# aperezhortal/pySPEEDY

Hardware: AMD Instinct MI355X
Metric: simulated-years/day (whole node), T30L8 (higher is better)
Workload: dtype f64

## Files before the change

### pyspeedy_amd/csrc/coupler_point.hpp

```cpp
#pragma once
#include <hip/hip_runtime.h>

#include "stream_store.hpp"
#include "surface.hpp"

namespace spd {

struct CouplerArgs {
    SurfacePtrs S;
    TimeInterp w;
    int first, count, day, land_coupling, sst_anomaly, anom_planes, fresh;
};

namespace cpl {
constexpr int NGc = IX * IL;
__device__ constexpr double SBCd = 5.67e-8f, ALHCd = 2501.0f, EMISFCd = 0.98f, ALBSEAd = 0.07f, ALBICEd = 0.60f;

__device__ inline double forin5(const double *f12, size_t p, const TimeInterp &w) {
    return w.w5[0] * f12[p + static_cast<size_t>(NGc) * w.m5[0]] + w.w5[1] * f12[p + static_cast<size_t>(NGc) * w.m5[1]] +
           w.w5[2] * f12[p + static_cast<size_t>(NGc) * w.m5[2]] + w.w5[3] * f12[p + static_cast<size_t>(NGc) * w.m5[3]] +
           w.w5[4] * f12[p + static_cast<size_t>(NGc) * w.m5[4]];
}
__device__ inline double forint(const double *f12, size_t p, const TimeInterp &w) {
    const double a = f12[p + static_cast<size_t>(NGc) * w.l0];
    const double d = w.wlin * (f12[p + static_cast<size_t>(NGc) * w.l1] - a);
    return a + d;
}
}


__device__ __forceinline__ void coupler_point(const SurfacePtrs &S, int mem, int p, const TimeInterp &w, int day, int land_coupling,
                                              int sst_anomaly, int anom_planes, int fresh) {
    using namespace cpl;
    constexpr int NG = NGc;
    const size_t o = static_cast<size_t>(mem) * NG + p, o12 = static_cast<size_t>(mem) * 12 * NG + p;
    double stlcl;
    if (fresh) {
        stlcl = forin5(S.stl12, o12, w);
        const double snowdcl = forint(S.snowd12, o12, w);
        const double soilwcl = forint(S.soilw12, o12, w);
        stream_store(&S.stlcl_obs[o], stlcl);
        stream_store(&S.snowdcl_obs[o], snowdcl);
        stream_store(&S.soilwcl_obs[o], soilwcl);
        stream_store(&S.snow_depth[o], snowdcl);
        stream_store(&S.soil_avail_water[o], soilwcl);
    } else {
        stlcl = S.stlcl_obs[o];
    }
    if (day == 0) {
        stream_store(&S.stl_lm[o], stlcl);
        stream_store(&S.land_temp[o], stlcl);
    } else if (land_coupling) {
        double tanom = S.stl_lm[o] - stlcl;
        tanom = S.cdland[o] * (tanom + S.rhcapl[o] * S.hfluxn[static_cast<size_t>(mem) * 3 * NG + p]);
        const double stl = tanom + stlcl;
        stream_store(&S.stl_lm[o], stl);
        stream_store(&S.land_temp[o], stl);
    } else if (fresh) {
        stream_store(&S.land_temp[o], stlcl);
    }

    const double sstfr = 273.2f - 1.8f;
    double sstcl, sicecl, ticecl, sstan_ob = S.sstan_ob[o];
    if (fresh) {
        sstcl = forin5(S.sst12, o12, w);
        sicecl = forint(S.sea_ice_frac12, o12, w);
        if (sst_anomaly) {
            const size_t oa = static_cast<size_t>(mem) * anom_planes * NG + p;
            const double a = S.sst_anom[oa + static_cast<size_t>(NG) * w.a0];
            const double da = w.wan * (S.sst_anom[oa + static_cast<size_t>(NG) * w.a1] - a);
            sstan_ob = a + da;
            stream_store(&S.sstan_ob[o], sstan_ob);
        }
        if (sstcl > sstfr) {
            sicecl = fmin(0.5, sicecl);
            ticecl = sstfr;
            if (sicecl > 0.0) sstcl = sstfr + (sstcl - sstfr) / (1.0f - sicecl);
        } else {
            sicecl = fmax(0.5, sicecl);
            ticecl = sstfr + (sstcl - sstfr) / sicecl;
            sstcl = sstfr;
        }
        stream_store(&S.sstcl_ob[o], sstcl);
        stream_store(&S.sicecl_ob[o], sicecl);
        stream_store(&S.ticecl_ob[o], ticecl);
    } else {
        sstcl = S.sstcl_ob[o];
        sicecl = S.sicecl_ob[o];
        ticecl = S.ticecl_ob[o];
    }
    double sst_om, tice_om, sice_om;
    if (day == 0) {
        sst_om = 0.0;
        tice_om = ticecl;
        sice_om = sicecl;
    } else {
        const double tice_am = S.tice_am[o], sice_am = S.sice_am[o];
        const double hfl2 = S.hfluxn[static_cast<size_t>(mem) * 3 * NG + NG + p];
        tice_om = S.tice_om[o];
        sst_om = S.sst_om[o];
        const double s4 = (sstfr * sstfr) * (sstfr * sstfr), t4 = (tice_am * tice_am) * (tice_am * tice_am);
        const double difice = (ALBSEAd - ALBICEd) * S.ssrd[o] + EMISFCd * SBCd * (s4 - t4) +
                              S.shf[static_cast<size_t>(mem) * 3 * NG + NG + p] + S.evap[static_cast<size_t>(mem) * 3 * NG + NG + p] * ALHCd;
        const double hflux_i = hfl2 + difice * (1.0f - sice_am);
        double hflux = hfl2 - S.hfseacl[o] - sicecl * (hflux_i + 1.0 * (sstfr - tice_om));
        double tanom = sst_om - sstcl;
        tanom = S.cdsea[o] * (tanom + S.rhcaps[o] * hflux);
        sst_om = tanom + sstcl;
        hflux = hflux_i + 1.0 * (sstfr - tice_om);
        tanom = tice_om - ticecl;
        const double anom0 = 20.f;
        const double cdis = S.cdice[o] * (anom0 / (anom0 + fabs(tanom)));
        tanom = cdis * (tanom + S.rhcapi[o] * hflux);
        tice_om = tanom + ticecl;
        sice_om = sicecl;
    }
    stream_store(&S.sst_om[o], sst_om);
    stream_store(&S.tice_om[o], tice_om);
    const double sstan_am = sst_anomaly ? sstan_ob : 0.0;
    if (fresh) {
        stream_store(&S.sice_om[o], sice_om);
        stream_store(&S.sstan_am[o], sstan_am);
        stream_store(&S.sice_am[o], sice_om);
    }
    double sst_am = sstcl + sstan_am;
    stream_store(&S.tice_am[o], tice_om);
    sst_am = sst_am + sice_om * (tice_om - sst_am);
    stream_store(&S.sst_am[o], sst_am);
    stream_store(&S.ssti_om[o], sst_om + sice_om * (tice_om - sst_om));
}

}
```

### pyspeedy_amd/csrc/dynamics.hip

```cpp
#include <hip/hip_runtime.h>

#include <type_traits>

#include "coupler_point.hpp"
#include "device_tables.hpp"
#include "diagnostics_block.hpp"
#include "dyn_column.hpp"
#include "launch_events.hpp"
#include "model.hpp"
#include "sppt_point.hpp"

namespace spd {

namespace {
using d2 = double __attribute__((ext_vector_type(2)));
constexpr int NG = IX * IL;
constexpr int kT = 256;

__device__ constexpr double CPd = 1004.0f;
__device__ constexpr double AKAPd = 2.0f / 7.0f;
__device__ constexpr double RGASd = AKAPd * CPd;
__device__ constexpr double WILd = 0.53f, TDRSd = 24.0f * 30.0f;

__device__ inline d2 times_i(d2 z) { return d2{-z.y, z.x}; }
// ... 94 lines not shown
}
template <int N>
__device__ inline double pick(const double (&a)[N], int l) {
    double r = a[0];
#pragma unroll
    for (int i = 1; i < N; ++i) r = (l == i) ? a[i] : r;
    return r;
}
template <int N>
__device__ inline d2 pick(const d2 (&a)[N], int l) {
    d2 r = a[0];
#pragma unroll
    for (int i = 1; i < N; ++i) r = (l == i) ? a[i] : r;
    return r;
}
}

struct NoCoupler {};
template <bool FOLD, bool EARLY, typename CA, int RIM = kRimPlain>
__global__ __launch_bounds__(kT) void spectral_step_kernel(ModelPtrs P, DeviceTables T, DynDeviceTables D, int M, int first,
                                                           int count, int j1, double dt, double eps, CA cpl, RimArg<RIM> rim) {
    static_assert(!FOLD || RIM == kRimPlain, "the folded form (small, latency-bound launches) has no rim modes");
    int nblocks = gridDim.x;
    if constexpr (std::is_same<CA, CouplerArgs>::value) {
        nblocks = (count * NSPEC * KX + kT - 1) / kT;
        if (static_cast<int>(blockIdx.x) >= nblocks) {
            const int gid = (blockIdx.x - nblocks) * kT + threadIdx.x;
            if (gid < cpl.count * NG) {
                const int lm = gid / NG;
                coupler_point(cpl.S, cpl.first + lm, gid - lm * NG, cpl.w, cpl.day, cpl.land_coupling, cpl.sst_anomaly,
                              cpl.anom_planes, cpl.fresh);
            }
            return;
        }
    }
    const int xcd = blockIdx.x & 7, q = nblocks >> 3, r = nblocks & 7;
    const int block = xcd * q + (xcd < r ? xcd : r) + (blockIdx.x >> 3);
    const int gid = block * kT + threadIdx.x;
    const int w = gid >> 6, lane = gid & 63;
    if (w >= count * kCoefBlocks) return;
    const int l = lane >> 3, kk = lane & 7;
    const int lm = w / kCoefBlocks, mem = first + lm, k = (w - lm * kCoefBlocks) * 8 + kk, n = k / MX, m = k - n * MX;
    if constexpr (RIM == kRimSkip) {
        if (tri::dead_block(w - lm * kCoefBlocks) && rim[mem] != 0) return;
    }
    unsigned seen = 0;
    auto note = [&](d2 v) {
        if constexpr (RIM == kRimDetect) {
            const unsigned long long x = __double_as_longlong(v.x) | __double_as_longlong(v.y);
            seen |= static_cast<unsigned>(x) | static_cast<unsigned>(x >> 32);
        }
    };
    const size_t f8 = static_cast<size_t>(mem) * 8 * NSPEC;
    const size_t fo = static_cast<size_t>(l) * NSPEC;
// ... 240 lines not shown
hipError_t run_dyn_grid(const ModelPtrs &P, const DynDeviceTables &D, int M, hipStream_t s) {
    launch(dyn_grid_kernel, dim3((M * NG + kT - 1) / kT), dim3(kT), 0, s, P, D, M);
    return hipGetLastError();
}
namespace {
template <bool FOLD, bool EARLY, typename CA, int RIM = kRimPlain>
void launch_spectral_step(dim3 grid, hipStream_t s, const ModelPtrs &P, const DeviceTables &T, const DynDeviceTables &D, int M,
                          int first, int count, int j1, double dt, double eps, const CA &cpl, RimArg<RIM> rim = {}) {
    launch(spectral_step_kernel<FOLD, EARLY, CA, RIM>, grid, dim3(kT), 0, s, P, T, D, M, first, count, j1, dt, eps, cpl, rim);
}
template <typename CA>
void dispatch_spectral_step(bool fold, bool early, int rim_mode, int *rim, dim3 grid, hipStream_t s, const ModelPtrs &P,
                            const DeviceTables &T, const DynDeviceTables &D, int M, int first, int count, int j1, double dt, double eps,
                            const CA &cpl) {
    if (fold && early) launch_spectral_step<true, true, CA>(grid, s, P, T, D, M, first, count, j1, dt, eps, cpl);
    else if (fold) launch_spectral_step<true, false, CA>(grid, s, P, T, D, M, first, count, j1, dt, eps, cpl);
    else if (rim_mode == kRimDetect && early) launch_spectral_step<false, true, CA, kRimDetect>(grid, s, P, T, D, M, first, count, j1, dt, eps, cpl, rim);
    else if (rim_mode == kRimDetect) launch_spectral_step<false, false, CA, kRimDetect>(grid, s, P, T, D, M, first, count, j1, dt, eps, cpl, rim);
    else if (rim_mode == kRimSkip && early) launch_spectral_step<false, true, CA, kRimSkip>(grid, s, P, T, D, M, first, count, j1, dt, eps, cpl, rim);
    else if (rim_mode == kRimSkip) launch_spectral_step<false, false, CA, kRimSkip>(grid, s, P, T, D, M, first, count, j1, dt, eps, cpl, rim);
    else if (early) launch_spectral_step<false, true, CA>(grid, s, P, T, D, M, first, count, j1, dt, eps, cpl);
    else launch_spectral_step<false, false, CA>(grid, s, P, T, D, M, first, count, j1, dt, eps, cpl);
}
}
hipError_t run_spectral_step(const ModelPtrs &P, const DeviceTables &T, const DynDeviceTables &D, int M, int first, int count,
                             int j1, double dt, double eps, const CouplerArgs *cpl, bool early, int rim_mode, int *rim, hipStream_t s) {
    const int nspec = (count * NSPEC * KX + kT - 1) / kT;
    const bool fold = P.phi_next != nullptr;
    if (fold && rim_mode != kRimPlain) return hipErrorInvalidValue;
    if (cpl)
        dispatch_spectral_step(fold, early, rim_mode, rim, dim3(nspec + (cpl->count * NG + kT - 1) / kT), s, P, T, D, M, first, count,
                               j1, dt, eps, *cpl);
    else
        dispatch_spectral_step(fold, early, rim_mode, rim, dim3(nspec), s, P, T, D, M, first, count, j1, dt, eps, NoCoupler{});
    return hipGetLastError();
}
hipError_t run_diagnostics(const ModelPtrs &P, const DeviceTables &T, int M, int tl, int *err, double *diag, int ticket,
                           hipStream_t s) {
    hipLaunchKernelGGL(diagnostics_kernel, dim3(M), dim3(64 * KX), 0, s, CheckArgs{P.vor, P.div, P.t, tl, err, diag, ticket}, T);
    return hipGetLastError();
}
hipError_t run_diagnostics_range(const ModelPtrs &P, const DeviceTables &T, int first, int count, int tl, int *err, double *diag,
                                 int ticket, hipStream_t s) {
    if (count <= 0) return hipSuccess;
    hipLaunchKernelGGL(diagnostics_kernel, dim3(count), dim3(64 * KX), 0, s, CheckArgs{P.vor, P.div, P.t, tl, err, diag, ticket, first}, T);
    return hipGetLastError();
}

}
```

### pyspeedy_amd/csrc/model.hip

```cpp
#include <dlfcn.h>
#include <hip/hip_runtime.h>

#include <algorithm>
#include <atomic>
#include <cassert>
#include <chrono>
#include <cmath>
#include <cstring>
#include <map>
#include <memory>
#include <mutex>
#include <string>
#include <thread>
#include <tuple>
#include <utility>
#include <vector>

#include "model_state.hpp"
#include "coupler_point.hpp"
#include "diagnostics_block.hpp"
#include "bounded_call.hpp"
#include "launch_events.hpp"
#include "sppt_point.hpp"
#include "staged_products.hpp"
#include "step_plan.hpp"
#include "stream_apart.hpp"

namespace spd {
hipError_t run_spec2grid_table(const DeviceTables &T, const FieldDesc *table, int nfields, hipStream_t st);
hipError_t run_grid2spec_table(const DeviceTables &T, const FieldDesc *table, int nfields, hipStream_t st);
hipError_t run_physics(const DeviceTables &T, const spd_physics_args &a, int nmembers, int fp32, hipStream_t s);
hipError_t run_dyn_physics(const ModelPtrs &P, const DynDeviceTables &D, const DeviceTables &T, const spd_physics_args &a,
                           int first, int nmembers, int fp32, int store32, int diag, double *tau_rec, int tau_store_record,
                           int tau_store_array, hipStream_t s);
hipError_t run_geopotential(const ModelPtrs &P, const DynDeviceTables &D, int first, int count, int tl, const SpptArgs *sppt,
                            int *rim, hipStream_t s);
hipError_t run_dyn_grid(const ModelPtrs &P, const DynDeviceTables &D, int M, hipStream_t s);
hipError_t run_spectral_step(const ModelPtrs &P, const DeviceTables &T, const DynDeviceTables &D, int M, int first, int count,
                             int j1, double dt, double eps, const CouplerArgs *cpl, bool early, int rim_mode, int *rim, hipStream_t s);
hipError_t run_diagnostics(const ModelPtrs &P, const DeviceTables &T, int M, int tl, int *err, double *diag, int ticket,
                           hipStream_t s);
hipError_t run_diagnostics_range(const ModelPtrs &P, const DeviceTables &T, int first, int count, int tl, int *err, double *diag,
                                 int ticket, hipStream_t s);
hipError_t run_coupler(const SurfacePtrs &S, int first, int count, const TimeInterp &w, int day, int land_coupling,
                       int sst_anomaly, int anom_planes, int fresh, hipStream_t s);
hipError_t run_forcing(const SurfacePtrs &S, int first, int count, const ZonalDevice &Z, double gamlat, double *corh_t,
                       double *corh_q, hipStream_t s);
hipError_t run_rest_state(const RestPtrs &R, int M, const RestConsts &c, hipStream_t s);
hipError_t run_scale_orog(const double *orog, double *phi0, long n, hipStream_t s);
hipError_t run_change_storage(double *array, long n, bool to_float, void *scratch, hipStream_t s);
hipError_t run_land_sea_init(const LandSeaPtrs &P, const LandSeaConsts &K, int first, int count, double *rows, hipStream_t s);
hipError_t run_multi_copy(const CopyList &L, hipStream_t s);
hipError_t run_spec2grid_table_check(const DeviceTables &T, const FieldDesc *table, int nfields, const CheckArgs &check, int members,
                                     hipStream_t st);
hipError_t run_copy_from_first(double *v, long n, int M, const int *flags, hipStream_t s);
hipError_t run_rest_surface(const double *phis0, double *forog, double *surf_ps, double *surf_q, const RestConsts &c, long n,
                            hipStream_t s);
hipError_t run_grid2spec(const DeviceTables &T, int stage, const double *src, double *dst, int prescale, int nfields,
                         hipStream_t stream);
hipError_t run_spec2grid(const DeviceTables &T, int stage, const double *src, double *dst, int kcos, int nfields,
                         hipStream_t stream);
hipError_t run_scale(const double *in, double *out, const double *table, double sign, int nfields, hipStream_t s);
// ... 456 lines not shown
        if (int rc = arena_alloc(owner, kDynSlabDoubles * sizeof(double), &p)) return rc;
        d = static_cast<double *>(p);
    }
    M_HIP(hipDeviceSynchronize());
    if (int rc = dyn_upload(ctx, *set, ctx->dyn_base.get(), d)) return rc;
    owner->dyn_private = std::move(set);
    *out = owner->dyn_private.get();
    return SPD_OK;
}

int spd_model_create(spd_handle h, int nmembers, spd_model_handle *out) {
    if (!h || !out) return m_fail(SPD_E_ARG, "spd_model_create: null argument");
    if (nmembers <= 0) return m_fail(SPD_E_ARG, "spd_model_create: nmembers must be positive");
    *out = nullptr;
    M_HIP(hipSetDevice(h->device));
    spd_model *m = new spd_model();
    m->ctx = h;
    m->M = nmembers;
    if (const char *env = getenv("PYSPEEDY_AMD_SPLIT_DYN")) m->split_dyn_physics = atoi(env) != 0;
    m->inv_per_member = 77;
    if (const char *env = getenv("PYSPEEDY_AMD_PRUNE_DEAD")) m->inv_per_member = atoi(env) != 0 ? 77 : 91;
    if (const char *env = getenv("PYSPEEDY_AMD_DIAG_EVERY_STEP")) m->diag_every_step = atoi(env) != 0;
    if (const char *env = getenv("PYSPEEDY_AMD_TAU_RECOMPUTE")) m->tau_recompute = atoi(env) < 0 || atoi(env) > 2 ? 1 : atoi(env);
    m->fold_geo = nmembers <= 8;
    if (const char *env = getenv("PYSPEEDY_AMD_SPECTRAL_EARLY")) m->spectral_early = atoi(env);
    if (const char *env = getenv("PYSPEEDY_AMD_FOLD_GEO")) m->fold_geo = atoi(env) != 0;
    if (const char *env = getenv("PYSPEEDY_AMD_PHYS_STORE32")) m->phys_store32 = atoi(env) != 0;
    m->nchunks = nmembers >= 64 ? 2 : (nmembers >= 24 ? 3 : (nmembers >= 20 ? 2 : 1));
    if (const char *env = getenv("PYSPEEDY_AMD_CHUNKS")) m->nchunks = atoi(env);
    if (m->nchunks < 1) m->nchunks = 1;
    if (m->nchunks > 4) m->nchunks = 4;
    if (m->nchunks > nmembers) m->nchunks = nmembers;
    if (const char *env = getenv("PYSPEEDY_AMD_BLOCK_MEMBERS")) m->block_members = atoi(env) > 0 ? atoi(env) : 0;
    const size_t M = nmembers, S = NSPEC * C, G3 = static_cast<size_t>(8) * NG;
    ModelPtrs &P = m->P;
    spd_physics_args &pa = m->pa;
    int rc = SPD_OK;
#define A(ptr, doubles, name, per)                      \
    if (rc == SPD_OK) rc = dalloc(m, (doubles), &(ptr), name, (per) * sizeof(double))
    A(P.vor, M * 2 * 8 * S, "vor", 2 * 8 * S);
    A(P.div, M * 2 * 8 * S, "div", 2 * 8 * S);
    A(P.t, M * 2 * 8 * S, "t", 2 * 8 * S);
    A(P.tr, M * 2 * 8 * S, "tr", 2 * 8 * S);
    A(P.ps, M * 2 * S, "ps", 2 * S);
    A(P.phi, M * 8 * S, "phi", 8 * S);
    A(m->phi_buf[1], M * 8 * S, nullptr, 0);
// ... 65 lines not shown
#undef PA_IN
#undef A
    if (rc != SPD_OK) {
        spd_model_destroy(m);
        return rc;
    }
    for (const char *name : {"t_grid_phys", "q_grid_phys", "phi_grid_phys", "pslg_phys", "u_grid_phys", "v_grid_phys",
                             "tt_rsw", "rad_tau2", "rad_strat_corr",
                             "rad_st4a", "rad_flux", "precnv", "precls", "cbmf", "slrd", "slr", "olr", "slru", "ustr", "vstr"})
        m->reg[name].f32 = true;
    if (rc == SPD_OK) {
        const spd_dyn_tables *base = nullptr;
        rc = dyn_tables(h, 0.0, nullptr, &base);
        if (rc == SPD_OK) m->D = base->dev;
    }
    if (rc == SPD_OK) {
        void *p = nullptr;
        rc = arena_alloc(m, sizeof(int) * M, &p);
        m->d_err = static_cast<int *>(p);
        if (rc == SPD_OK) rc = arena_alloc(m, sizeof(double) * M * 24, &p);
        m->d_diag = static_cast<double *>(p);
        if (rc == SPD_OK) rc = arena_alloc(m, sizeof(int) * M, &p);
        m->d_rim = static_cast<int *>(p);
    }
    if (rc == SPD_OK) rc = build_tables(m);
    if (rc != SPD_OK) {
        spd_model_destroy(m);
        return rc;
    }
    *out = m;
    return SPD_OK;
}

int spd_model_destroy(spd_model_handle m) {
    if (!m) return SPD_OK;
    (void)hipSetDevice(m->ctx->device);
    constexpr size_t kIdleBytes = static_cast<size_t>(1) << 30;
    bool keep_first = false;
    if (!m->blocks.empty() && hipDeviceSynchronize() == hipSuccess) {
        std::lock_guard<std::mutex> lock(m->ctx->idle_mutex);
        if (m->ctx->idle_bytes + m->blocks[0].size <= kIdleBytes) {
            m->ctx->idle_blocks.push_back({m->blocks[0].base, m->blocks[0].size});
            m->ctx->idle_bytes += m->blocks[0].size;
            keep_first = true;
        }
    }
// ... 188 lines not shown
};

static bool folds(const spd_model *m) { return m->fold_geo && !m->nudge.loops() && !m->assim.loops(); }

static bool begin_step_geopotential(spd_model *m) {
    const bool fold = folds(m);
    const bool ahead = fold && m->phi_ahead;
    if (ahead) m->phi_cur ^= 1;
    m->P.phi = m->phi_buf[m->phi_cur];
    m->P.phi_next = fold ? m->phi_buf[m->phi_cur ^ 1] : nullptr;
    m->reg["phi"].ptr = m->P.phi;
    m->phi_ahead = fold;
    return !ahead;
}

static void sppt_advance(spd_model *m) {
    if (!m->sppt_on) return;
    m->sppt_first = false;
    m->sppt_step += 1;
}

static bool staged_products(const spd_model *m) { return !(m->split_dyn_physics && !m->phys_fp32); }

static hipError_t step_range(spd_model *m, int j1, int j2, double dt, int compute_shortwave, int first, int count, int diag,
                             bool run_geo, const CouplerArgs *cpl, hipStream_t s, hipEvent_t after_grid2spec = nullptr,
                             const CheckArgs *ride = nullptr, int rim_mode = kRimPlain, const TauPlan &tau = TauPlan{}) {
    const DeviceTables &T = m->ctx->dev;
    const int M = m->M;
    hipError_t e = hipSuccess;
    if (m->fail_launch_after >= 0 && m->fail_launch_after-- == 0) return hipErrorLaunchFailure;
    SpptArgs sp{};
    if (m->sppt_on)
        sp = sppt_args(m->sppt_spec + static_cast<size_t>(first) * 8 * NSPEC * C, T, count, m->sppt_seed, m->sppt_member_base + first,
                       m->sppt_step, m->sppt_first ? 1 : 0);
    if (run_geo) {
        ProfScope ps(m, SPD_K_GEOPOTENTIAL, count, s);
        e = run_geopotential(m->P, m->D, first, count, 0, m->sppt_on ? &sp : nullptr, rim_mode == kRimSkip ? m->d_rim : nullptr,
                             s);
    } else if (m->sppt_on) {
        ProfScope ps(m, SPD_K_SPPT, 8 * count, s);
        e = run_sppt_update(sp, s);
    }
    spd_physics_args pa = m->pa;
    pa.compute_shortwave = compute_shortwave ? 1 : 0;
    pa.air_absortivity_co2 = m->air_absortivity_co2;
    pa.sppt_pattern = m->sppt_on ? m->sppt_grid : nullptr;
    if (e == hipSuccess) {
        const int per = m->inv_per_member + (m->sppt_on ? 8 : 0);
        FieldDesc *table = (m->stored32 ? (m->sppt_on ? m->inv_table_sppt32 : m->inv_table32)
// ... 18 lines not shown
            {
                ProfScope ps(m, SPD_K_DYN_GRID, M, s);
                e = run_dyn_grid(m->P, m->D, M, s);
            }
            if (e == hipSuccess) {
                ProfScope ps(m, compute_shortwave ? SPD_K_PHYSICS_SW : SPD_K_PHYSICS, M, s);
                e = run_physics(T, pa, M, m->phys_fp32, s);
            }
        } else {
            ProfScope ps(m, compute_shortwave ? SPD_K_COLUMN_SW : SPD_K_COLUMN, count, s);
            e = run_dyn_physics(m->P, m->D, T, pa, first, count, m->phys_fp32, m->stored32 ? 1 : 0, diag, tau.compact ? m->tau_rec : nullptr,
                                tau.store_record ? 1 : 0, tau.store_array ? 1 : 0, s);
        }
    }
    if (e == hipSuccess) {
        ProfScope ps(m, SPD_K_GRID2SPEC, 73 * count, s);
        const FieldDesc *fwd = staged_products(m) ? m->fwd_table_products : m->fwd_table;
        e = run_grid2spec_table(T, fwd + static_cast<size_t>(first) * 73, 73 * count, s);
    }
    if (after_grid2spec && e == hipSuccess) e = hipEventRecord(after_grid2spec, s);
    const double eps = (j1 == 1) ? 0.0 : static_cast<double>(0.05f);
    if (e == hipSuccess) {
        ProfScope ps(m, SPD_K_SPECTRAL_STEP, count, s);
        const bool early = m->spectral_early < 0 ? count <= 8 : m->spectral_early != 0;
        e = run_spectral_step(m->P, T, m->D, M, first, count, j1 - 1, dt, eps, cpl, early, rim_mode, m->d_rim, s);
    }
    return e;
}

int spd_model_step_dynamics(spd_model_handle m, int j1, int j2, double dt, int compute_shortwave, void *stream) {
    if (!m) return m_fail(SPD_E_ARG, "spd_model_step_dynamics: null model");
    if (j1 < 1 || j1 > 2 || j2 < 1 || j2 > 2) return m_fail(SPD_E_ARG, "spd_model_step_dynamics: time levels are 1 or 2");
    if (!m->dyn) return m_fail(SPD_E_ARG, "spd_model_step_dynamics: call spd_model_set_time_step first");
    if (int rc = settle_deferred_check(m)) return rc;
    const bool run_geo = begin_step_geopotential(m);
    const hipError_t e = step_range(m, j1, j2, dt, compute_shortwave, 0, m->M, 1, run_geo, nullptr, static_cast<hipStream_t>(stream));
    if (e != hipSuccess) return m_fail(SPD_E_DEVICE, std::string("spd_model_step_dynamics: ") + hipGetErrorString(e));
    sppt_advance(m);
    return SPD_OK;
}

static int next_ticket(spd_model *m) {
    m->check_ticket = m->check_ticket % 0x0fffffff + 1;
    return m->check_ticket;
}

static int wait_codes(spd_model *m, const int *pinned, int ticket, hipEvent_t ev, hipStream_t s, int32_t *out, const char *who) {
    const volatile int *codes = pinned;
// ... 301 lines not shown
        m->groups_apart = m->groups_apart && apart;
        M_HIP(hipEventCreateWithFlags(&m->cev[g], hipEventDisableTiming));
    }
    return SPD_OK;
}


static auto host_state(spd_model *m) {
    return std::tie(m->cal, m->current_step, m->phi_cur, m->surf_cache_valid, m->phi_ahead, m->sppt_first, m->sppt_step, m->air_absortivity_co2);
}
using HostState = std::tuple<Calendar, int, int, bool, bool, bool, long long, double>;

struct OpenWindows { int acc_start; WinOpen win; };

struct Segment {
    spd_model *m;
    int nsteps;
    bool record;
    const char *who;
    int row0;
    hipStream_t gs[kGroupStreams];
    Partition part;
    bool offset, rim, tau_compact;
    int c0;
    double tau_co2;
    HostState start;
    long long nudged0;
    SampleCursor stats, tape, spectra, enstape, acctape, wintape, projtape;
    OpenWindows open0, open;
    int rc = SPD_OK;
    bool launched, device_failed;
    void check_launch(hipError_t e, const char *feature) {
        if (e == hipSuccess) return;
        (void)hipGetLastError();
        rc = m_fail(SPD_E_DEVICE, std::string(who) + ": " + feature + hipGetErrorString(e));
        device_failed = true;
    }
    void note_accepted(int row) const {
        if (!record) return;
        int32_t *a = m->steps_accepted.data() + 7 * static_cast<size_t>(row0 + row);
        stamp_row(a, m->current_step, m->cal);
        a[6] = m->cal.month_idx;
    }
    void rewind() {
        for (SampleCursor *c : {&stats, &tape, &spectra, &enstape, &acctape, &wintape, &projtape}) c->rewind();
        open = open0;
    }
};

static const char kSstUncovered[] = "SST anomaly planes do not cover the simulated period (speedy.py:338-372)";
static bool sst_anomaly_covered(const spd_model *m, const TimeInterp &w) {
    return !m->sst_anomaly_flag || (w.a0 >= 0 && w.a1 >= 0 && w.a0 < m->anom_planes && w.a1 < m->anom_planes);
}

static int plan_segment(Segment &sg) {
    spd_model *m = sg.m;
    sg.rim = sg.nsteps >= 2 && !folds(m);
    m->rim_call = sg.rim;
    sg.start = host_state(m);
    sg.c0 = m->current_step;
    sg.tau_compact = m->tau_recompute != 0 && sg.nsteps > 1 && staged_products(m);
    if ((sg.part.rounds > 1 || sg.tau_compact) && m->sst_anomaly_flag) {
        Calendar ahead = m->cal;
        for (int it = 0; it < sg.nsteps; ++it) {
            ahead.advance();
            if (!sst_anomaly_covered(m, time_interp(ahead))) {
                if (sg.part.rounds > 1) return m_fail(SPD_E_ARG, kSstUncovered);
                sg.tau_compact = false;
            }
        }
    }
    sg.nudged0 = m->nudge.applied;
    sg.stats = SampleCursor(m->stats.samples);
    sg.tape = SampleCursor(m->tape.ring.taken);
    sg.spectra = SampleCursor(m->spectra.ring.taken);
    sg.enstape = SampleCursor(m->enstape.ring.taken);
    sg.projtape = SampleCursor(m->projtape.ring.taken);
    spd_model::AccTape &ac = m->acctape;
    if (ac.on && (ac.window_start < 0 || ac.window_start > m->current_step)) ac.window_start = m->current_step;
    sg.acctape = SampleCursor(ac.ring.taken);
    spd_model::WinTape &wt = m->wintape;
    if (wt.on && (wt.window_start < 0 || wt.window_start > m->current_step)) {
        wt.window_start = m->current_step;
        wt.samples = 0;
    }
    sg.wintape = SampleCursor(wt.ring.taken);
    sg.open0 = OpenWindows{ac.window_start, WinOpen{wt.window_start, wt.samples}};
    return SPD_OK;
}

struct StepPlan {
    bool new_day;
    ZonalDevice zd;
    int sw, diag, fresh;
    long long stats_n, tape_n, spectra_n, enstape_n, projtape_n;
    bool fold_enstape, acc_close, run_geo;
    int acc_step, acc_slot;
    WinDecision win;
    WinOpen win_after;
    int32_t win_row[8];
    int win_k, win_n, win_slot;
    TauPlan tau;
    Calendar next;
    TimeInterp w;
};

static StepPlan decide_step(Segment &sg, int round, int it) {
    spd_model *m = sg.m;
    const spd_model::AccTape &ac = m->acctape;
    const spd_model::WinTape &wt = m->wintape;
    const int c = m->current_step;
    StepPlan p{};
    p.new_day = c % 36 == 0;
    if (p.new_day) p.zd = forcing_host(m, 1);
    p.sw = (c % 3 == 0) ? 1 : 0;
    if (m->stats.on && due_after(c, m->stats.every)) p.stats_n = sg.stats.next();
    if (m->tape.on && due_after(c, m->tape.every)) p.tape_n = sg.tape.next();
// ... 5 lines not shown
    if (p.fold_enstape && round == 0) {
        int *held = m->enstape.counts.data() + kEnsTapeGroups * static_cast<size_t>(m->enstape.ring.slot(p.enstape_n));
        std::fill(held, held + kEnsTapeGroups, 0);
    }
    p.acc_step = c + 1 - sg.open.acc_start;
    p.acc_close = ac.on && due_after(c, ac.every);
    if (ac.on) p.acc_slot = ac.ring.slot(sg.acctape.open());
    p.next = m->cal;
    p.next.advance();
    p.win_after = sg.open.win;
    if (wt.on) p.win = wintape_advance(WinSchedule{wt.window, wt.every, wt.sample_every}, p.win_after, c + 1, p.next, p.win_row);
    p.win_k = p.win.sample ? sg.open.win.samples + 1 : 0;
    p.win_n = sg.open.win.samples + (p.win.sample ? 1 : 0);
    if (p.win.sample || p.win.close) p.win_slot = wt.ring.slot(sg.wintape.open());
    if (m->projtape.on && due_after(c, m->projtape.every)) p.projtape_n = sg.projtape.next();
    p.diag = (m->diag_every_step || it == sg.nsteps - 1 || (p.stats_n && m->stats.precip) || (p.tape_n && m->tape.precip) ||
              (p.fold_enstape && m->enstape.precip) || ac.on || (p.win.sample && wt.precip) || (p.projtape_n && m->projtape.precip)) ? 1 : 0;
    p.w = time_interp(p.next);
    p.fresh = (!m->surf_cache_valid || (p.next.hour == 0 && p.next.minute == 0)) ? 1 : 0;
    if (!sst_anomaly_covered(m, p.w)) {
        sg.rc = m_fail(SPD_E_ARG, kSstUncovered);
        return p;
    }
    const bool tau_round = sg.tau_compact && (m->tau_recompute == 2 || sg.part.round_count(round) >= kTauFromMembers);
    p.tau = tau_plan(tau_round, p.sw != 0, it, sg.nsteps, tau_first_sw(sg.c0), m->diag_every_step);
    if (p.tau.store_record) sg.tau_co2 = m->air_absortivity_co2;
    else if (p.tau.compact) assert(m->air_absortivity_co2 == sg.tau_co2);
    p.run_geo = begin_step_geopotential(m);
    return p;
}

static void issue_group(Segment &sg, const StepPlan &p, int round, int it, int g, int first, int count) {
    spd_model *m = sg.m;
    const spd_model::Nudge &nd = m->nudge;
    const spd_model::AccTape &ac = m->acctape;
    hipStream_t s = sg.gs[g];
    const bool record = sg.record, first_of_call = it == 0 && round == 0;
    const double delt = 86400.0 / 36;
    const int tl_check = 1;
    sg.launched = true;
    if (p.new_day && (sg.rc = forcing_range(m, p.zd, first, count, s)) != SPD_OK) sg.device_failed = true;
    CouplerArgs cpl{m->S, p.w, first, count, 1 + (m->current_step + 1) / 36, m->land_coupling_flag, m->sst_anomaly_flag, m->anom_planes,
                    p.fresh};
    if (sg.rc == SPD_OK) {
        hipError_t e = hipSuccess;
        if (sg.offset && first_of_call && g == 1) e = hipStreamWaitEvent(s, m->ev_offset, 0);
        if (sg.rim && it == 0 && e == hipSuccess)
            e = hipMemsetD32Async(reinterpret_cast<hipDeviceptr_t>(m->d_rim + first), 1, static_cast<size_t>(count), s);
        const CheckArgs chk{m->P.vor, m->P.div, m->P.t, tl_check, record && it > 0 ? m->h_steps_err + static_cast<size_t>(sg.row0 + it - 1) * m->M : nullptr,
                            nullptr, m->steps_ticket, first};
        if (e == hipSuccess)
            e = step_range(m, 2, 2, 2 * delt, p.sw, first, count, p.diag, p.run_geo, &cpl, s,
                           (sg.offset && first_of_call && g == 0) ? m->ev_offset : nullptr, record && it > 0 ? &chk : nullptr,
                           sg.rim ? (it == 0 ? kRimDetect : kRimSkip) : kRimPlain, p.tau);
        sg.check_launch(e, "");
    }
    if (sg.rc == SPD_OK && nd.loops()) {
        const NudgeAt at = nudge_at(nd.stamps, m->current_step + 1);
        sg.check_launch(run_nudge(nd.planes, nd.nplanes, nd.mask, first, count, at.s0, at.s1, at.a, s), "nudging: ");
    }
    if (sg.rc == SPD_OK && record && it == sg.nsteps - 1) {
        sg.check_launch(run_diagnostics_range(m->P, m->ctx->dev, first, count, tl_check, m->h_steps_err + static_cast<size_t>(sg.row0 + it) * m->M,
                                              nullptr, m->steps_ticket, s), "");
        ++m->checks_alone;
    }
    if (sg.rc == SPD_OK && p.stats_n)
        sg.check_launch(stats_sample(m, first, count, p.stats_n, s), "time statistics: ");
    if (sg.rc == SPD_OK && p.tape_n)
        sg.check_launch(tape_sample(m, first, count, p.tape_n, s), "tape: ");
    if (sg.rc == SPD_OK && p.spectra_n)
        sg.check_launch(spectra_sample(m, first, count, p.spectra_n, s), "spectra: ");
    if (sg.rc == SPD_OK && p.fold_enstape)
        sg.check_launch(enstape_sample(m, first, count, p.enstape_n, g, s), "ensemble tape: ");
    if (sg.rc == SPD_OK && ac.on)
        sg.check_launch(run_acctape_step(ac.planes, ac.nplanes, first, count, p.acc_step, p.acc_close ? 1 : 0, p.acc_slot, m->stored32 ? 1 : 0,
                                         ac.dtype == SPD_TAPE_F64 ? 1 : 0, s),
                        "accumulation tape: ");
    if (sg.rc == SPD_OK && (p.win.sample || p.win.close))
        sg.check_launch(wintape_step(m, first, count, p.win_k, p.win.close ? 1 : 0, p.win_n, p.win_slot, s), "window tape: ");
    if (sg.rc == SPD_OK && p.projtape_n)
        sg.check_launch(projtape_sample(m, first, count, p.projtape_n, s), "projection tape: ");
}

static void commit_step(Segment &sg, const StepPlan &p, bool first_round, int it) {
    spd_model *m = sg.m;
    sppt_advance(m);
    m->current_step += 1;
    m->cal = p.next;
    m->surf_cache_valid = true;
    if (first_round) sg.note_accepted(it + 1);
    if (first_round && m->nudge.loops()) m->nudge.applied = sg.nudged0 + it + 1;
    if (first_round && p.stats_n) m->stats.samples = sg.stats.last();
    if (p.tape_n) sg.tape.commit(m->tape.ring, first_round, m->current_step, p.next);
    if (p.spectra_n) sg.spectra.commit(m->spectra.ring, first_round, m->current_step, p.next);
    if (p.enstape_n) sg.enstape.commit(m->enstape.ring, first_round, m->current_step, p.next);
    if (p.projtape_n) sg.projtape.commit(m->projtape.ring, first_round, m->current_step, p.next);
    if (p.acc_close) {
        spd_model::AccTape &ac = m->acctape;
        sg.acctape.next();
        sg.open.acc_start = m->current_step;
        sg.acctape.commit(ac.ring, first_round, m->current_step, p.next);
        if (first_round) ac.window_start = sg.open.acc_start;
        if (first_round) ac.ring.row(ac.ring.taken)[6] = p.acc_step;
    }
    spd_model::WinTape &wt = m->wintape;
    sg.open.win = p.win_after;
    if (p.win.close) sg.wintape.next();
    if (wt.on && first_round) {
        wt.window_start = sg.open.win.start;
        wt.samples = sg.open.win.samples;
        if (p.win.close) {
            sg.wintape.commit(wt.ring, true, m->current_step, p.next);
// ... 328 lines not shown
}

int spd_model_get_option(spd_model_handle m, const char *name, int32_t *value) {
    if (!m || !name || !value) return m_fail(SPD_E_ARG, "spd_model_get_option: null argument");
    const std::string key(name);
    if (key == "diag_every_step") *value = m->diag_every_step ? 1 : 0;
    else if (key == "split_dyn") *value = m->split_dyn_physics ? 1 : 0;
    else if (key == "spectral_early") *value = m->spectral_early;
    else if (key == "member_groups") *value = m->nchunks;
    else if (key == "block_members") *value = m->block_members;
    else if (key == "physics_storage32") *value = m->phys_store32 ? 1 : 0;
    else if (key == "tau_recompute") *value = m->tau_recompute;
    else if (key == "staged_products") *value = staged_products(m) ? 1 : 0;
    else if (key == "quiet_rim_members") {
        *value = -1;
        if (m->rim_call) {
            std::vector<int> flags(static_cast<size_t>(m->M));
            M_HIP(hipDeviceSynchronize());
            M_HIP(hipMemcpy(flags.data(), m->d_rim, sizeof(int) * flags.size(), hipMemcpyDeviceToHost));
            *value = 0;
            for (int f : flags) *value += f != 0 ? 1 : 0;
        }
    }
    else return m_fail(SPD_E_ARG, "spd_model_get_option: unknown option: " + key);
    return SPD_OK;
}

int spd_model_set_option(spd_model_handle m, const char *name, int32_t value) {
    if (!m || !name) return m_fail(SPD_E_ARG, "spd_model_set_option: null argument");
    const std::string key(name);
    const bool flag = value == 0 || value == 1;
    if (key == "diag_every_step" && flag) m->diag_every_step = value != 0;
    else if (key == "split_dyn" && flag) m->split_dyn_physics = value != 0;
    else if (key == "tau_recompute" && value >= 0 && value <= 2) m->tau_recompute = value;
    else if (key == "spectral_early" && value >= -1 && value <= 1) m->spectral_early = value;
    else if (key == "member_groups" && value >= 1 && value <= 4) m->nchunks = value < m->M ? value : m->M;
    else if (key == "block_members" && value >= 0) m->block_members = value;
    else if (key == "fail_launch_after" && value >= -1) m->fail_launch_after = value;
    else if (key == "prepare_multi_step" && value == 1) {
        if (int rc = ensure_steps_record(m, 360)) return rc;
        if (m->nchunks > 1 && !m->split_dyn_physics) return ensure_group_streams(m, m->nchunks);
    }
    else if (key == "physics_storage32" && flag) {
        m->phys_store32 = value != 0;
        return apply_storage(m, m->phys_fp32 && m->phys_store32);
    }
    else return m_fail(SPD_E_ARG, "spd_model_set_option: unknown option or value out of range: " + key);
    return SPD_OK;
}

int spd_model_set_flags(spd_model_handle m, int land_coupling_flag, int sst_anomaly_coupling_flag, int increase_co2) {
    if (!m) return m_fail(SPD_E_ARG, "spd_model_set_flags: null model");
    m->land_coupling_flag = land_coupling_flag ? 1 : 0;
    m->sst_anomaly_flag = sst_anomaly_coupling_flag ? 1 : 0;
    m->increase_co2 = increase_co2 ? 1 : 0;
    m->surf_cache_valid = false;
    return SPD_OK;
}
// ... 355 lines not shown
```

### pyspeedy_amd/csrc/model_state.hpp

```cpp
#pragma once
#include <hip/hip_runtime.h>

#include <algorithm>
#include <cmath>
#include <cstring>
#include <map>
#include <memory>
#include <string>
#include <utility>
#include <vector>

#include "../../include/pyspeedy_amd.h"
#include "context.hpp"
#include "model.hpp"
#include "plev.hpp"
#include "derive.hpp"
#include "stats.hpp"
#include "spectra.hpp"
#include "tape.hpp"
#include "enstape.hpp"
#include "acctape.hpp"
#include "nudge.hpp"
#include "breed.hpp"
#include "assim.hpp"
// ... 23 lines not shown
    const spd_dyn_tables *dyn = nullptr;
    std::unique_ptr<spd_dyn_tables> dyn_private;
    DynDeviceTables D{};
    spd_physics_args pa{};
    struct Block {
        char *base;
        size_t size, used;
    };
    std::vector<Block> blocks;
    std::map<std::string, RegEntry> reg;
    FieldDesc *inv_table[2][2] = {{nullptr, nullptr}, {nullptr, nullptr}};
    FieldDesc *inv_table_sppt[2][2] = {{nullptr, nullptr}, {nullptr, nullptr}};
    FieldDesc *inv_table32[2][2] = {{nullptr, nullptr}, {nullptr, nullptr}}, *inv_table_sppt32[2][2] = {{nullptr, nullptr}, {nullptr, nullptr}};
    FieldDesc *fwd_table = nullptr;
    FieldDesc *fwd_table_products = nullptr;
    double *phi_buf[2] = {nullptr, nullptr};
    int phi_cur = 0;
    bool phi_ahead = false, fold_geo = true;
    bool groups_apart = true;
    int *d_err = nullptr;
    double *d_diag = nullptr;
    int *d_rim = nullptr;
    bool rim_call = false;
    int *h_err[2] = {nullptr, nullptr}, *h_err_sync = nullptr;
    hipEvent_t err_event[2] = {nullptr, nullptr};
    int next_slot = 0;
    bool slot_busy[2] = {false, false};
    int check_ticket = 0, slot_ticket[2] = {0, 0};
    struct DeferredCheck {
        bool active = false;
        int slot = -1, time_level = 2;
        hipStream_t stream = nullptr;
    } deferred;
    hipStream_t slot_stream[2] = {nullptr, nullptr};
    bool slot_rode[2] = {false, false};
    int checks_alone = 0, checks_rode = 0;
    double air_absortivity_co2 = 6.0;
    SurfacePtrs S{};
    Calendar cal;
    int current_step = 0;
    bool initialized = false;
    bool sppt_on = false, sppt_first = true;
    unsigned long long sppt_seed = 0;
    long long sppt_member_base = 0, sppt_step = 0;
    double *sppt_spec = nullptr, *sppt_grid = nullptr;
    int inv_per_member = 77;
// ... 374 lines not shown
```

### pyspeedy_amd/csrc/step_plan.hpp

```cpp
#pragma once

namespace spd {

constexpr int kGroupStreams = 4;

struct Partition {
    int M = 1, G = 1, rounds = 1;
    int round_count(int r) const { return M / rounds + (r < M % rounds ? 1 : 0); }
    int group_count(int n, int g) const { return n / G + (g < n % G ? 1 : 0); }
};
inline Partition partition_members(int M, int nchunks, int block_members, int nsteps, bool one_group) {
    Partition p;
    p.M = M;
    p.G = (one_group || nsteps == 1) ? 1 : nchunks;
    const bool may_round = p.G > 1 || (nchunks == 1 && !one_group);
    if (may_round && nsteps > 1 && block_members > 0 && M >= 4 * block_members)
        p.rounds = (M + p.G * block_members - 1) / (p.G * block_members);
    return p;
}

constexpr int kTauFromMembers = 20;
struct TauPlan {
    bool compact = false;
    bool store_record = false, store_array = false;
};
inline int tau_first_sw(int c0) { return ((3 - c0 % 3) % 3 + 3) % 3; }
inline TauPlan tau_plan(bool takes_part, bool sw, int it, int nsteps, int first_sw, bool diag_every_step) {
    TauPlan tau;
    if (takes_part && sw && it != nsteps - 1) {
        tau.compact = tau.store_record = true;
        tau.store_array = it + 3 > nsteps - 1 || diag_every_step;
    } else if (takes_part && !sw && it > first_sw) {
        tau.compact = true;
    }
    return tau;
}

inline bool due_after(int c, int every) { return (c + 1) % every == 0; }
inline bool enstape_folds(long long n, long long taken0, int c0, int nsteps, int every, int capacity) {
    const long long last = taken0 + (static_cast<long long>(c0) + nsteps) / every - c0 / every;
    return n + capacity > last;
}

}
```

Baseline: 1.888 million.

## Share identical per-member surface planes in coupler via verify-then-shared reads

Adds a verify form of the ocean/land coupler that compares each member's climatology and coefficient planes bitwise against the group's first member and records a per-member 'same' flag. On later non-fresh steps, the shared form reads those planes from the reference member when the flag is set, so identical ensemble members hit the same cache lines instead of streaming separate copies. It adds a memset and extra comparison loads on verify steps, plus new template instantiations and control logic, in exchange for reduced memory traffic on shared steps. The path is enabled by default when partitioning permits.

```diff
diff --git a/pyspeedy_amd/csrc/coupler_point.hpp b/pyspeedy_amd/csrc/coupler_point.hpp
--- a/pyspeedy_amd/csrc/coupler_point.hpp
+++ b/pyspeedy_amd/csrc/coupler_point.hpp
@@ -1,5 +1,7 @@
 #pragma once
 #include <hip/hip_runtime.h>
+
+#include <type_traits>
 
 #include "stream_store.hpp"
 #include "surface.hpp"
@@ -11,6 +13,17 @@
     TimeInterp w;
     int first, count, day, land_coupling, sst_anomaly, anom_planes, fresh;
 };
+
+constexpr int kCplOwn = 0, kCplVerify = 1, kCplShared = 2;
+struct CouplerVerifyArgs : CouplerArgs {
+    int *same;
+};
+struct CouplerSharedArgs : CouplerArgs {
+    int *same;
+};
+template <typename CA>
+constexpr int coupler_form_of = std::is_same<CA, CouplerVerifyArgs>::value ? kCplVerify
+                                : std::is_same<CA, CouplerSharedArgs>::value ? kCplShared : kCplOwn;
 
 namespace cpl {
 constexpr int NGc = IX * IL;
@@ -26,14 +39,29 @@
     const double d = w.wlin * (f12[p + static_cast<size_t>(NGc) * w.l1] - a);
     return a + d;
 }
+__device__ inline unsigned long long bit_difference(const double *plane, size_t o, size_t oref) {
+    return static_cast<unsigned long long>(__double_as_longlong(plane[o]) ^ __double_as_longlong(plane[oref]));
+}
 }
 
 
+template <int FORM = kCplOwn>
 __device__ __forceinline__ void coupler_point(const SurfacePtrs &S, int mem, int p, const TimeInterp &w, int day, int land_coupling,
-                                              int sst_anomaly, int anom_planes, int fresh) {
+                                              int sst_anomaly, int anom_planes, int fresh, int ref = 0, int *same = nullptr) {
     using namespace cpl;
     constexpr int NG = NGc;
     const size_t o = static_cast<size_t>(mem) * NG + p, o12 = static_cast<size_t>(mem) * 12 * NG + p;
+    if constexpr (FORM != kCplOwn) fresh = 0;
+    size_t os = o;
+    if constexpr (FORM == kCplVerify) {
+        const size_t oref = static_cast<size_t>(ref) * NG + p;
+        unsigned long long d = 0;
+        for (const double *plane : {S.stlcl_obs, S.sstcl_ob, S.sicecl_ob, S.ticecl_ob, S.sstan_ob, S.sice_am, S.cdland, S.rhcapl,
+                                    S.hfseacl, S.cdsea, S.rhcaps, S.cdice, S.rhcapi})
+            d |= bit_difference(plane, o, oref);
+        if (d != 0) same[mem] = 0;
+    }
+    if constexpr (FORM == kCplShared) os = static_cast<size_t>(same[mem] != 0 ? ref : mem) * NG + p;
     double stlcl;
     if (fresh) {
         stlcl = forin5(S.stl12, o12, w);
@@ -45,14 +73,14 @@
         stream_store(&S.snow_depth[o], snowdcl);
         stream_store(&S.soil_avail_water[o], soilwcl);
     } else {
-        stlcl = S.stlcl_obs[o];
+        stlcl = S.stlcl_obs[os];
     }
     if (day == 0) {
         stream_store(&S.stl_lm[o], stlcl);
         stream_store(&S.land_temp[o], stlcl);
     } else if (land_coupling) {
         double tanom = S.stl_lm[o] - stlcl;
-        tanom = S.cdland[o] * (tanom + S.rhcapl[o] * S.hfluxn[static_cast<size_t>(mem) * 3 * NG + p]);
+        tanom = S.cdland[os] * (tanom + S.rhcapl[os] * S.hfluxn[static_cast<size_t>(mem) * 3 * NG + p]);
         const double stl = tanom + stlcl;
         stream_store(&S.stl_lm[o], stl);
         stream_store(&S.land_temp[o], stl);
@@ -61,7 +89,7 @@
     }
 
     const double sstfr = 273.2f - 1.8f;
-    double sstcl, sicecl, ticecl, sstan_ob = S.sstan_ob[o];
+    double sstcl, sicecl, ticecl, sstan_ob = S.sstan_ob[os];
     if (fresh) {
         sstcl = forin5(S.sst12, o12, w);
         sicecl = forint(S.sea_ice_frac12, o12, w);
@@ -85,9 +113,9 @@
         stream_store(&S.sicecl_ob[o], sicecl);
         stream_store(&S.ticecl_ob[o], ticecl);
     } else {
-        sstcl = S.sstcl_ob[o];
-        sicecl = S.sicecl_ob[o];
-        ticecl = S.ticecl_ob[o];
+        sstcl = S.sstcl_ob[os];
+        sicecl = S.sicecl_ob[os];
+        ticecl = S.ticecl_ob[os];
     }
     double sst_om, tice_om, sice_om;
     if (day == 0) {
@@ -95,7 +123,7 @@
         tice_om = ticecl;
         sice_om = sicecl;
     } else {
-        const double tice_am = S.tice_am[o], sice_am = S.sice_am[o];
+        const double tice_am = S.tice_am[o], sice_am = S.sice_am[os];
         const double hfl2 = S.hfluxn[static_cast<size_t>(mem) * 3 * NG + NG + p];
         tice_om = S.tice_om[o];
         sst_om = S.sst_om[o];
@@ -103,15 +131,15 @@
         const double difice = (ALBSEAd - ALBICEd) * S.ssrd[o] + EMISFCd * SBCd * (s4 - t4) +
                               S.shf[static_cast<size_t>(mem) * 3 * NG + NG + p] + S.evap[static_cast<size_t>(mem) * 3 * NG + NG + p] * ALHCd;
         const double hflux_i = hfl2 + difice * (1.0f - sice_am);
-        double hflux = hfl2 - S.hfseacl[o] - sicecl * (hflux_i + 1.0 * (sstfr - tice_om));
+        double hflux = hfl2 - S.hfseacl[os] - sicecl * (hflux_i + 1.0 * (sstfr - tice_om));
         double tanom = sst_om - sstcl;
-        tanom = S.cdsea[o] * (tanom + S.rhcaps[o] * hflux);
+        tanom = S.cdsea[os] * (tanom + S.rhcaps[os] * hflux);
         sst_om = tanom + sstcl;
         hflux = hflux_i + 1.0 * (sstfr - tice_om);
         tanom = tice_om - ticecl;
         const double anom0 = 20.f;
-        const double cdis = S.cdice[o] * (anom0 / (anom0 + fabs(tanom)));
-        tanom = cdis * (tanom + S.rhcapi[o] * hflux);
+        const double cdis = S.cdice[os] * (anom0 / (anom0 + fabs(tanom)));
+        tanom = cdis * (tanom + S.rhcapi[os] * hflux);
         tice_om = tanom + ticecl;
         sice_om = sicecl;
     }
diff --git a/pyspeedy_amd/csrc/dynamics.hip b/pyspeedy_amd/csrc/dynamics.hip
--- a/pyspeedy_amd/csrc/dynamics.hip
+++ b/pyspeedy_amd/csrc/dynamics.hip
@@ -140,14 +140,21 @@
                                                            int count, int j1, double dt, double eps, CA cpl, RimArg<RIM> rim) {
     static_assert(!FOLD || RIM == kRimPlain, "the folded form (small, latency-bound launches) has no rim modes");
     int nblocks = gridDim.x;
-    if constexpr (std::is_same<CA, CouplerArgs>::value) {
+    if constexpr (std::is_base_of<CouplerArgs, CA>::value) {
         nblocks = (count * NSPEC * KX + kT - 1) / kT;
         if (static_cast<int>(blockIdx.x) >= nblocks) {
             const int gid = (blockIdx.x - nblocks) * kT + threadIdx.x;
             if (gid < cpl.count * NG) {
-                const int lm = gid / NG;
-                coupler_point(cpl.S, cpl.first + lm, gid - lm * NG, cpl.w, cpl.day, cpl.land_coupling, cpl.sst_anomaly,
-                              cpl.anom_planes, cpl.fresh);
+                if constexpr (std::is_same<CA, CouplerArgs>::value) {
+                    const int lm = gid / NG;
+                    coupler_point(cpl.S, cpl.first + lm, gid - lm * NG, cpl.w, cpl.day, cpl.land_coupling, cpl.sst_anomaly,
+                                  cpl.anom_planes, cpl.fresh);
+                } else {
+                    static_assert(NG % kT == 0, "a coupling block never straddles members");
+                    const int um = __builtin_amdgcn_readfirstlane(static_cast<int>(blockIdx.x - nblocks) / (NG / kT));
+                    coupler_point<coupler_form_of<CA>>(cpl.S, cpl.first + um, gid - um * NG, cpl.w, cpl.day, cpl.land_coupling,
+                                                       cpl.sst_anomaly, cpl.anom_planes, 0, cpl.first, cpl.same);
+                }
             }
             return;
         }
@@ -434,13 +441,27 @@
     else if (early) launch_spectral_step<false, true, CA>(grid, s, P, T, D, M, first, count, j1, dt, eps, cpl);
     else launch_spectral_step<false, false, CA>(grid, s, P, T, D, M, first, count, j1, dt, eps, cpl);
 }
+template <typename CA>
+void dispatch_shared_planes(int rim_mode, int *rim, dim3 grid, hipStream_t s, const ModelPtrs &P, const DeviceTables &T,
+                            const DynDeviceTables &D, int M, int first, int count, int j1, double dt, double eps, const CA &cpl) {
+    if (rim_mode == kRimDetect) launch_spectral_step<false, false, CA, kRimDetect>(grid, s, P, T, D, M, first, count, j1, dt, eps, cpl, rim);
+    else if (rim_mode == kRimSkip) launch_spectral_step<false, false, CA, kRimSkip>(grid, s, P, T, D, M, first, count, j1, dt, eps, cpl, rim);
+    else launch_spectral_step<false, false, CA>(grid, s, P, T, D, M, first, count, j1, dt, eps, cpl);
+}
 }
 hipError_t run_spectral_step(const ModelPtrs &P, const DeviceTables &T, const DynDeviceTables &D, int M, int first, int count,
-                             int j1, double dt, double eps, const CouplerArgs *cpl, bool early, int rim_mode, int *rim, hipStream_t s) {
+                             int j1, double dt, double eps, const CouplerArgs *cpl, bool early, int rim_mode, int *rim, hipStream_t s,
+                             int cpl_form, int *same) {
     const int nspec = (count * NSPEC * KX + kT - 1) / kT;
     const bool fold = P.phi_next != nullptr;
     if (fold && rim_mode != kRimPlain) return hipErrorInvalidValue;
-    if (cpl)
+    if (cpl_form != kCplOwn && (!cpl || fold || early || !same || cpl->fresh)) return hipErrorInvalidValue;
+    const dim3 with_coupling(nspec + (cpl ? (cpl->count * NG + kT - 1) / kT : 0));
+    if (cpl_form == kCplVerify)
+        dispatch_shared_planes(rim_mode, rim, with_coupling, s, P, T, D, M, first, count, j1, dt, eps, CouplerVerifyArgs{*cpl, same});
+    else if (cpl_form == kCplShared)
+        dispatch_shared_planes(rim_mode, rim, with_coupling, s, P, T, D, M, first, count, j1, dt, eps, CouplerSharedArgs{*cpl, same});
+    else if (cpl)
         dispatch_spectral_step(fold, early, rim_mode, rim, dim3(nspec + (cpl->count * NG + kT - 1) / kT), s, P, T, D, M, first, count,
                                j1, dt, eps, *cpl);
     else
diff --git a/pyspeedy_amd/csrc/model.hip b/pyspeedy_amd/csrc/model.hip
--- a/pyspeedy_amd/csrc/model.hip
+++ b/pyspeedy_amd/csrc/model.hip
@@ -37,7 +37,8 @@
                             int *rim, hipStream_t s);
 hipError_t run_dyn_grid(const ModelPtrs &P, const DynDeviceTables &D, int M, hipStream_t s);
 hipError_t run_spectral_step(const ModelPtrs &P, const DeviceTables &T, const DynDeviceTables &D, int M, int first, int count,
-                             int j1, double dt, double eps, const CouplerArgs *cpl, bool early, int rim_mode, int *rim, hipStream_t s);
+                             int j1, double dt, double eps, const CouplerArgs *cpl, bool early, int rim_mode, int *rim, hipStream_t s,
+                             int cpl_form = kCplOwn, int *same = nullptr);
 hipError_t run_diagnostics(const ModelPtrs &P, const DeviceTables &T, int M, int tl, int *err, double *diag, int ticket,
                            hipStream_t s);
 hipError_t run_diagnostics_range(const ModelPtrs &P, const DeviceTables &T, int first, int count, int tl, int *err, double *diag,
@@ -540,6 +541,7 @@
     if (const char *env = getenv("PYSPEEDY_AMD_PRUNE_DEAD")) m->inv_per_member = atoi(env) != 0 ? 77 : 91;
     if (const char *env = getenv("PYSPEEDY_AMD_DIAG_EVERY_STEP")) m->diag_every_step = atoi(env) != 0;
     if (const char *env = getenv("PYSPEEDY_AMD_TAU_RECOMPUTE")) m->tau_recompute = atoi(env) < 0 || atoi(env) > 2 ? 1 : atoi(env);
+    if (const char *env = getenv("PYSPEEDY_AMD_SHARED_PLANES")) m->shared_planes = atoi(env) != 0 ? 1 : 0;
     m->fold_geo = nmembers <= 8;
     if (const char *env = getenv("PYSPEEDY_AMD_SPECTRAL_EARLY")) m->spectral_early = atoi(env);
     if (const char *env = getenv("PYSPEEDY_AMD_FOLD_GEO")) m->fold_geo = atoi(env) != 0;
@@ -651,6 +653,8 @@
         m->d_diag = static_cast<double *>(p);
         if (rc == SPD_OK) rc = arena_alloc(m, sizeof(int) * M, &p);
         m->d_rim = static_cast<int *>(p);
+        if (rc == SPD_OK) rc = arena_alloc(m, sizeof(int) * M, &p);
+        m->d_same = static_cast<int *>(p);
     }
     if (rc == SPD_OK) rc = build_tables(m);
     if (rc != SPD_OK) {
@@ -885,9 +889,12 @@
 
 static bool staged_products(const spd_model *m) { return !(m->split_dyn_physics && !m->phys_fp32); }
 
+static_assert(static_cast<int>(CouplerForm::own) == kCplOwn && static_cast<int>(CouplerForm::verify) == kCplVerify &&
+              static_cast<int>(CouplerForm::shared) == kCplShared, "step_plan.hpp and coupler_point.hpp name the same forms");
 static hipError_t step_range(spd_model *m, int j1, int j2, double dt, int compute_shortwave, int first, int count, int diag,
                              bool run_geo, const CouplerArgs *cpl, hipStream_t s, hipEvent_t after_grid2spec = nullptr,
-                             const CheckArgs *ride = nullptr, int rim_mode = kRimPlain, const TauPlan &tau = TauPlan{}) {
+                             const CheckArgs *ride = nullptr, int rim_mode = kRimPlain, const TauPlan &tau = TauPlan{},
+                             CouplerForm form = CouplerForm::own) {
     const DeviceTables &T = m->ctx->dev;
     const int M = m->M;
     hipError_t e = hipSuccess;
@@ -952,8 +959,9 @@
     const double eps = (j1 == 1) ? 0.0 : static_cast<double>(0.05f);
     if (e == hipSuccess) {
         ProfScope ps(m, SPD_K_SPECTRAL_STEP, count, s);
-        const bool early = m->spectral_early < 0 ? count <= 8 : m->spectral_early != 0;
-        e = run_spectral_step(m->P, T, m->D, M, first, count, j1 - 1, dt, eps, cpl, early, rim_mode, m->d_rim, s);
+        const bool early = m->spectral_early < 0 ? count <= kEarlyMembers : m->spectral_early != 0;
+        e = run_spectral_step(m->P, T, m->D, M, first, count, j1 - 1, dt, eps, cpl, early, rim_mode, m->d_rim, s, static_cast<int>(form),
+                              m->d_same);
     }
     return e;
 }
@@ -1301,6 +1309,7 @@
     hipStream_t gs[kGroupStreams];
     Partition part;
     bool offset, rim, tau_compact;
+    bool share, fresh_before;
     int c0;
     double tau_co2;
     HostState start;
@@ -1324,6 +1333,7 @@
     void rewind() {
         for (SampleCursor *c : {&stats, &tape, &spectra, &enstape, &acctape, &wintape, &projtape}) c->rewind();
         open = open0;
+        fresh_before = false;
     }
 };
 
@@ -1336,6 +1346,8 @@
     spd_model *m = sg.m;
     sg.rim = sg.nsteps >= 2 && !folds(m);
     m->rim_call = sg.rim;
+    sg.share = m->shared_planes != 0 && shares_planes(sg.part, sg.nsteps, folds(m), m->spectral_early);
+    m->same_call = false;
     sg.start = host_state(m);
     sg.c0 = m->current_step;
     sg.tau_compact = m->tau_recompute != 0 && sg.nsteps > 1 && staged_products(m);
@@ -1372,6 +1384,7 @@
     bool new_day;
     ZonalDevice zd;
     int sw, diag, fresh;
+    CouplerForm form;
     long long stats_n, tape_n, spectra_n, enstape_n, projtape_n;
     bool fold_enstape, acc_close, run_geo;
     int acc_step, acc_slot;
@@ -1423,6 +1436,7 @@
         sg.rc = m_fail(SPD_E_ARG, kSstUncovered);
         return p;
     }
+    p.form = coupler_form(sg.share, p.fresh != 0, sg.fresh_before, it, sg.nsteps);
     const bool tau_round = sg.tau_compact && (m->tau_recompute == 2 || sg.part.round_count(round) >= kTauFromMembers);
     p.tau = tau_plan(tau_round, p.sw != 0, it, sg.nsteps, tau_first_sw(sg.c0), m->diag_every_step);
     if (p.tau.store_record) sg.tau_co2 = m->air_absortivity_co2;
@@ -1448,12 +1462,14 @@
         if (sg.offset && first_of_call && g == 1) e = hipStreamWaitEvent(s, m->ev_offset, 0);
         if (sg.rim && it == 0 && e == hipSuccess)
             e = hipMemsetD32Async(reinterpret_cast<hipDeviceptr_t>(m->d_rim + first), 1, static_cast<size_t>(count), s);
+        if (p.form == CouplerForm::verify && e == hipSuccess)
+            e = hipMemsetD32Async(reinterpret_cast<hipDeviceptr_t>(m->d_same + first), 1, static_cast<size_t>(count), s);
         const CheckArgs chk{m->P.vor, m->P.div, m->P.t, tl_check, record && it > 0 ? m->h_steps_err + static_cast<size_t>(sg.row0 + it - 1) * m->M : nullptr,
                             nullptr, m->steps_ticket, first};
         if (e == hipSuccess)
             e = step_range(m, 2, 2, 2 * delt, p.sw, first, count, p.diag, p.run_geo, &cpl, s,
                            (sg.offset && first_of_call && g == 0) ? m->ev_offset : nullptr, record && it > 0 ? &chk : nullptr,
-                           sg.rim ? (it == 0 ? kRimDetect : kRimSkip) : kRimPlain, p.tau);
+                           sg.rim ? (it == 0 ? kRimDetect : kRimSkip) : kRimPlain, p.tau, p.form);
         sg.check_launch(e, "");
     }
     if (sg.rc == SPD_OK && nd.loops()) {
@@ -1489,6 +1505,8 @@
     m->current_step += 1;
     m->cal = p.next;
     m->surf_cache_valid = true;
+    sg.fresh_before = p.fresh != 0;
+    m->same_call = p.form != CouplerForm::own;
     if (first_round) sg.note_accepted(it + 1);
     if (first_round && m->nudge.loops()) m->nudge.applied = sg.nudged0 + it + 1;
     if (first_round && p.stats_n) m->stats.samples = sg.stats.last();
@@ -1863,6 +1881,17 @@
             for (int f : flags) *value += f != 0 ? 1 : 0;
         }
     }
+    else if (key == "shared_planes") *value = m->shared_planes;
+    else if (key == "shared_plane_members") {
+        *value = -1;
+        if (m->same_call) {
+            std::vector<int> flags(static_cast<size_t>(m->M));
+            M_HIP(hipDeviceSynchronize());
+            M_HIP(hipMemcpy(flags.data(), m->d_same, sizeof(int) * flags.size(), hipMemcpyDeviceToHost));
+            *value = 0;
+            for (int f : flags) *value += f != 0 ? 1 : 0;
+        }
+    }
     else return m_fail(SPD_E_ARG, "spd_model_get_option: unknown option: " + key);
     return SPD_OK;
 }
@@ -1875,6 +1904,7 @@
     else if (key == "split_dyn" && flag) m->split_dyn_physics = value != 0;
     else if (key == "tau_recompute" && value >= 0 && value <= 2) m->tau_recompute = value;
     else if (key == "spectral_early" && value >= -1 && value <= 1) m->spectral_early = value;
+    else if (key == "shared_planes" && flag) m->shared_planes = value;
     else if (key == "member_groups" && value >= 1 && value <= 4) m->nchunks = value < m->M ? value : m->M;
     else if (key == "block_members" && value >= 0) m->block_members = value;
     else if (key == "fail_launch_after" && value >= -1) m->fail_launch_after = value;
diff --git a/pyspeedy_amd/csrc/model_state.hpp b/pyspeedy_amd/csrc/model_state.hpp
--- a/pyspeedy_amd/csrc/model_state.hpp
+++ b/pyspeedy_amd/csrc/model_state.hpp
@@ -69,6 +69,9 @@
     double *d_diag = nullptr;
     int *d_rim = nullptr;
     bool rim_call = false;
+    int *d_same = nullptr;
+    int shared_planes = 1;
+    bool same_call = false;
     int *h_err[2] = {nullptr, nullptr}, *h_err_sync = nullptr;
     hipEvent_t err_event[2] = {nullptr, nullptr};
     int next_slot = 0;
diff --git a/pyspeedy_amd/csrc/step_plan.hpp b/pyspeedy_amd/csrc/step_plan.hpp
--- a/pyspeedy_amd/csrc/step_plan.hpp
+++ b/pyspeedy_amd/csrc/step_plan.hpp
@@ -36,6 +36,19 @@
     return tau;
 }
 
+enum class CouplerForm { own, verify, shared };
+inline CouplerForm coupler_form(bool takes_part, bool fresh, bool fresh_before, int it, int nsteps) {
+    if (!takes_part || fresh || nsteps < 2) return CouplerForm::own;
+    if (it == 0 || fresh_before) return it == nsteps - 1 ? CouplerForm::own : CouplerForm::verify;
+    return CouplerForm::shared;
+}
+constexpr int kEarlyMembers = 8;
+inline bool shares_planes(const Partition &p, int nsteps, bool folds, int spectral_early) {
+    const int smallest = p.group_count(p.round_count(p.rounds - 1), p.G - 1);
+    const bool early = spectral_early < 0 ? smallest <= kEarlyMembers : spectral_early != 0;
+    return nsteps >= 2 && !folds && !early && smallest > 0;
+}
+
 inline bool due_after(int c, int every) { return (c + 1) % every == 0; }
 inline bool enstape_folds(long long n, long long taken0, int c0, int nsteps, int every, int capacity) {
     const long long last = taken0 + (static_cast<long long>(c0) + nsteps) / every - c0 / every;
```

Result: no change. 1.895 million, median of 6 (+0.4%).
